# itailang/SampleNet

Measured on AMD Instinct MI355X. Metric: point-clouds/sec fwd+bwd, Bx1024->64 soft-proj+Chamfer, higher is better.
Workload: dtype f32; 1 GPU; BASELINE configs[1]: SampleNet sampler train step (fwd + simplification/projection losses + bwd), B=32 per GPU, 1024->64 points, K=8, bottleneck 128; no optimizer step; batch_per_gpu=32, global_batch=32, n_in=1024, n_out=64, group_size=8, parallelism=dp1, rccl_ranks=0, grad_allreduce=none, execution=whole step replayed as one hipGraph

## Files before the change

### include/samplenet_hip_internal.h

```cpp
#ifndef SAMPLENET_HIP_INTERNAL_H
#define SAMPLENET_HIP_INTERNAL_H

#include "samplenet_hip.h"

#ifdef __cplusplus
extern "C" {
#endif

int sn_sampler_loss_forward(int nproj, const float *proj, const float *lsimp, const float *temperature,
                            float alpha, float lmbda, float min_sigma, float *loss, sn_stream_t stream);
int sn_sampler_loss_backward(int nproj, const float *grad_loss, const float *temperature, float alpha, float lmbda,
                             float min_sigma, float *grad_proj, float *grad_lsimp, float *grad_T, sn_stream_t stream);

int sn_pairscan_colmin_splits(int B, int N, int M);
int sn_pairscan_forward_partial(int B, int N, int M, int K, const float *P, int p_layout, const float *Q, int q_layout,
                                int *knn_idx, float *dist_q, int *idx_q, float *proj, int proj_layout,
                                const float *temperature, float min_sigma, void *workspace, long long workspace_bytes,
                                sn_stream_t stream);
int sn_pairscan_forward_partial_fc(int B, int N, int M, int K, const float *P, int p_layout, const float *fc_z,
                                   const float *fc_scale, const float *fc_shift, const float *fc_w, const float *fc_bias,
                                   int Kfc, float *q_out, int *knn_idx, float *dist_q, int *idx_q, float *proj,
                                   int proj_layout, const float *temperature, float min_sigma, void *workspace,
                                   long long workspace_bytes, sn_stream_t stream);
int sn_sampler_step_loss_forward(int B, int M, int N, int G, const float *dist_q, const void *colmin_ws, const float *proj,
                                 const float *temperature, float alpha, float lmbda, float weight, float min_sigma,
                                 float *dist_p, int *idx_p, int *argmax1, float *partial, float *loss, int defer_value,
                                 sn_stream_t stream);
int sn_sampler_step_loss_forward_direct(int B, int M, int N, const float *dist_q, const float *dist_p, const float *proj,
                                        const float *temperature, float alpha, float lmbda, float weight, float min_sigma,
                                        int *argmax1, float *partial, float *loss, int defer_value, sn_stream_t stream);
int sn_sampler_step_loss_backward(int B, int N, int M, int K, const float *P, int p_layout, const float *Q,
                                  const int *knn_idx, const int *idx_q, const int *idx_p, const int *argmax1,
                                  const float *temperature, float min_sigma, float alpha, float lmbda, float weight,
                                  const float *grad_loss, float *grad_Q, float *gsig_scratch, float *grad_T,
                                  const float *deferred_partial, float *deferred_loss, sn_stream_t stream);
int sn_pairscan_forward_keys(int B, int N, int M, int K, const float *P, int p_layout, float *Q, const float *fc_z,
                             const float *fc_scale, const float *fc_shift, const float *fc_w, const float *fc_bias, int Kfc,
                             int *knn_idx, float *dist_q, int *idx_q, float *proj, int proj_layout, const float *temperature,
                             float min_sigma, void *colmin_keys, float *qpart, void *qmax, sn_stream_t stream);
int sn_sampler_step_loss_keys(int B, int N, int M, int K, const float *P, int p_layout, const float *Q, const int *knn_idx,
                              const int *idx_q, void *colmin_keys, const float *qpart, const void *qmax, int G,
                              const float *temperature, float min_sigma, float alpha, float lmbda, float weight,
                              const float *grad_loss, float *grad_Q, float *gsig_scratch, float *grad_T, float *dpsum,
                              float *loss, sn_stream_t stream, void *deferred_tail, const float *grad_proj,
                              const float *grad_sigma);
int sn_surface_values_keys(int B, int N, int M, int G, const void *colmin_keys, const float *qpart, const void *qmax,
                           const float *temperature, float min_sigma, float weight, const float *y_bcn, float *simp_bnc,
                           float *dpsum, float *values, sn_stream_t stream);
int sn_surface_gather_upstream(int nproj, const float *g_lsimp, const float *g_sigma, const float *g_proj, float *scalars,
                               float *proj_out, sn_stream_t stream);
int sn_conv_stack_set_persist_min_tiles(int tiles);
int sn_fps_set_variant(int v);
int sn_step_tail_bytes(void);
int sn_step_tail_set_error_words(void *tail_blob, const void *fwd_sync, const void *bwd_sync);


int sn_layer_forward_bn(int R, int Ci, int Co, const float *ain, const float *coef_prev, const float *W,
                        const float *bias, float *z, float *stats, const float *gamma, const float *beta,
                        float eps, float momentum, float *running_mean, float *running_var,
                        long long *num_batches_tracked, float *coef, sn_stream_t stream);
int sn_conv_forward_bn_pool(int R, int Ci, int Co, int npts, const float *ain, const float *coef_prev, const float *W,
                            const float *bias, float *z, float *stats, const float *gamma, const float *beta, float eps,
                            float momentum, float *running_mean, float *running_var, long long *num_batches_tracked,
                            float *coef, float *pool_val, int *pool_idx, float *pooled, int *argsel, float *zsel,
                            sn_stream_t stream);
int sn_conv_stack_forward_supported(int B, int N, int nlayers, const int *channels);
long long sn_conv_stack_acc_elems(int nlayers);
int sn_conv_stack_z1_free_supported(int B, int N, int nlayers, const int *channels);
long long sn_conv_stack_acc_sum_elems(int nlayers, const int *channels);
int sn_conv_stack_forward_bn(int B, int N, int nlayers, const int *channels, const float *x, const float *const *W,
                             const float *const *bias, const float *const *gamma, const float *const *beta,
                             float *const *running_mean, float *const *running_var, long long *const *num_batches_tracked,
                             const float *eps, const float *momentum, float *const *z, float *const *coef, long long *acc,
                             float *pool_val, int *pool_idx, float *pooled, int *argsel, float *zsel, sn_stream_t stream);
long long sn_conv_stack_backward_scratch_floats(int B, int N, int nlayers, const int *channels);
int sn_conv_stack_backward(int B, int N, int nlayers, const int *channels, const float *x, const float *const *W,
                           const float *bias0, const float *const *z, const float *const *coef, const float *gsel,
                           const int *argsel, const float *kcoef_top, long long *acc, float *scratch, float *const *dW,
                           float *const *dgamma, float *const *dbeta, float *const *dbias, const void *step_tail,
                           sn_stream_t stream);
int sn_layer_backward(int R, int Ci, int Co, int dz_mode, const float *dy, const float *z, const float *kcoef,
                      const float *gsel, const int *argsel, int npts, const float *W, const float *zprev,
                      const float *coef_prev, float *dyprev, float *stats, float *part, float *dW, float *db,
                      float *prev_dgamma, float *prev_dbeta, float *prev_dbias, float *prev_kcoef, long long prev_bn_rows,
// ... 220 lines not shown
```

### samplenet_amd/csrc/pointnet_mlp.hip

```cpp
#include "mlp_host.h"

namespace sn {

template <class T, bool FULL, int AMODE, int KT = 0, bool PLANES = false, bool IN3A = false>
__global__ void __launch_bounds__(T::THREADS) __attribute__((amdgpu_waves_per_eu(T::THREADS / 128, 8))) linear_fwd_kernel(FwdArgs g)
{
    extern __shared__ __attribute__((aligned(16))) float lds[];
    SN_TL(0);
    SN_TL_ID(0);
    const int row0 = blockIdx.x * T::BM, col0 = blockIdx.y * T::BN;
    const int R = g.a.rows, Co = g.w.co, Ci = g.w.ci;
    f32x16 acc[T::TM][T::TN];
#pragma unroll
    for (int i = 0; i < T::TM; ++i)
#pragma unroll
        for (int j = 0; j < T::TN; ++j)
#pragma unroll
            for (int e = 0; e < 16; ++e) acc[i][j][e] = 0.f;
    const ActSrc a = g.a;
    const WSrc w = g.w;
    const int lane = threadIdx.x & 63;
    const int wave = __builtin_amdgcn_readfirstlane(threadIdx.x >> 6);
    const int wr = wave / T::WC, wc = wave % T::WC;
    float biasv[T::TN];
// ... 1465 lines not shown
    return 1;
}

[[maybe_unused]] constexpr long long kWPlaneLL = (long long)128 * 128 * 3 * 2 / 8;
[[maybe_unused]] constexpr long long kWPlaneWideLL = (long long)256 * 256 * 3 * 2 / 8;
static bool conv_stack_wide(int nlayers, const int *channels)
{
    for (int l = 1; l <= nlayers; ++l)
        if (channels[l] > kFxRow) return true;
    return false;
}
extern "C" int sn_conv_stack_z1_free_supported(int B, int N, int nlayers, const int *channels)
{
#if SN_BF16X3
    if (!sn_conv_stack_forward_supported(B, N, nlayers, channels) || nlayers < 3 || nlayers - 1 > 4) return 0;
    if (channels[1] != 64 || channels[2] != 64) return 0;
    long long nb = 0;
    for (int l = 1; l < nlayers; ++l) nb += ((long long)channels[l] * channels[l + 1] + 1023) / 1024;
    return nb <= (long long)B * N / 64 ? 1 : 0;
#else
    return 0;
#endif
}
extern "C" long long sn_conv_stack_acc_sum_elems(int nlayers, const int *channels)
{
    if (nlayers <= 0) return 0;
    return (long long)nlayers * ((channels && conv_stack_wide(nlayers, channels)) ? 2 : 1) * kFxLayer;
}
extern "C" long long sn_conv_stack_acc_elems(int nlayers)
{
    return nlayers > 0 ? (long long)nlayers * 2 * kFxLayer + (long long)(nlayers - 1) * kWPlaneWideLL : 0;
}

static int g_persist_min_tiles = 4;
static int g_in3_blocks = 0;
extern "C" int sn_conv_stack_set_in3_blocks(int blocks)
{
    const int prev = g_in3_blocks;
    g_in3_blocks = blocks < 0 ? 0 : blocks;
    return prev;
}
extern "C" int sn_conv_stack_set_persist_min_tiles(int tiles)
{
    const int old = g_persist_min_tiles;
    g_persist_min_tiles = tiles;
    return old;
}
template <class TT, int KT, bool IN3A>
static int launch_fwd_persist(const FwdArgs &g, int ntiles, int tpw, int nwg, hipStream_t st)
{
    const size_t lds = sizeof(float) * ((size_t)(KT / BKX) * 3 * TT::BM * LDX + 2 * KT + (size_t)2 * TT::WR * 2 * TT::BN + (size_t)TT::WR * TT::WC * 16 * 36);
    static SnLdsAttr attr;
    if (sn_lds_attr(attr, (const void *)linear_fwd_persist_kernel<TT, KT, IN3A, 2>, lds, "linear_fwd_persist_kernel")) return SN_ERR_UNSUPPORTED;
    hipLaunchKernelGGL((linear_fwd_persist_kernel<TT, KT, IN3A, 2>), dim3(nwg), dim3(TT::THREADS), lds, st, g, ntiles, tpw);
    return 0;
}

template <class TT, int KT>
static void launch_fwd_fx(const FwdArgs &g, dim3 grid, size_t lds, hipStream_t st)
{
    if (g.wplanes)
        hipLaunchKernelGGL((linear_fwd_kernel<TT, true, ACT_BN_RELU_FX, KT, SN_BF16X3 != 0>), grid, dim3(TT::THREADS), lds, st, g);
    else
        hipLaunchKernelGGL((linear_fwd_kernel<TT, true, ACT_BN_RELU_FX, KT>), grid, dim3(TT::THREADS), lds, st, g);
}

extern "C" int sn_conv_stack_forward_bn(int B, int N, int nlayers, const int *channels, const float *x, const float *const *W,
                                        const float *const *bias, const float *const *gamma, const float *const *beta,
                                        float *const *running_mean, float *const *running_var,
                                        long long *const *num_batches_tracked, const float *eps, const float *momentum,
                                        float *const *z, float *const *coef, long long *acc, float *pool_val, int *pool_idx,
                                        float *pooled, int *argsel, float *zsel, sn_stream_t stream)
{
    if (!sn_conv_stack_forward_supported(B, N, nlayers, channels))
        return sn_set_error(SN_ERR_UNSUPPORTED, "sn_conv_stack_forward_bn: needs N % 64 == 0 and 64 / 128 (/ 256 inside the stack) channels");
    SN_REQUIRE(x && W && gamma && beta && eps && momentum && z && coef && acc && pool_val && pool_idx, "null pointer");
    SN_REQUIRE((pooled && argsel && zsel) || (!pooled && !argsel && !zsel), "pooled / argsel / zsel: all or none");
    hipStream_t st = (hipStream_t)stream;
// ... 27 lines not shown
        if (nb > R / 64) job.n = 0;
    }
#endif
    const bool keys_pool = !pooled || (B > 32 && N >= 128 && channels[nlayers] <= 128);
    if (keys_pool) {
        job.zero_keys = reinterpret_cast<unsigned long long *>(pool_val), job.nkeys = B * 2 * channels[nlayers];
        SN_REQUIRE((long long)job.nkeys <= (long long)(R / 64) * 256, "too few rows to clear the pool keys");
    }
    int in3_nb = 1;
    {
        const long long need = std::max<long long>(job.n > 0 ? job.first[job.n] : 0, keys_pool ? (job.nkeys + 255) / 256 : 0);
        while (in3_nb < 8 && (R / 64) / (in3_nb * 2) >= std::max<long long>(need, 4 * device_cus()) && (R / 64) % (in3_nb * 2) == 0) in3_nb *= 2;
        if (g_in3_blocks > 0 && (R / 64) / g_in3_blocks >= std::max<long long>(need, 1)) in3_nb = g_in3_blocks;
    }
    hipLaunchKernelGGL(conv_in3_fwd_kernel, dim3((R / 64 + in3_nb - 1) / in3_nb, channels[1] / 64), dim3(256), 0, st, R, channels[1], x, W[0],
                       bias ? bias[0] : nullptr, z[0], (float *)nullptr, acc, acc + (size_t)(nlayers - 1) * S + kFxPoison, job,
                       in3_nb);
    using T = TileBig;
    for (int l = 1; l < nlayers; ++l) {
        const int Ci = channels[l], Co = channels[l + 1];
        FwdArgs g = make_fwd(R, Ci, Co, z[l - 1], nullptr, W[l], bias ? bias[l] : nullptr, z[l], nullptr);
        g.acc_in = acc + (size_t)(l - 1) * S, g.bn_prev = bn_of(l - 1), g.acc_out = acc + (size_t)l * S;
        if (l >= 2) g.zero_ptr = acc + (size_t)(l - 2) * S, g.zero_n = (int)S;
        if (l == nlayers - 1) {
            g.pool_npts = N;
            if (!keys_pool) g.pool_val = pool_val, g.pool_idx = pool_idx;
            else g.pool_keys = reinterpret_cast<unsigned long long *>(pool_val);
        }
        g.wplanes = job.n > 0 ? planes[l] : nullptr;
        const bool pl = g.wplanes != nullptr;
#if SN_BF16X3
        if (pl && g.z && (l < nlayers - 1 || keys_pool) && (l > 1 || z1free) && (Ci == 64 || Co == 128) && Ci <= 128 && Co <= 128 && R % 64 == 0) {
            const int ntiles = R / 64, per_cu = Co == 128 ? 1 : 2, nmax = device_cus() * per_cu;
            if (g_persist_min_tiles > 0 && ntiles >= g_persist_min_tiles * nmax) {
                const int tpw = (ntiles + nmax - 1) / nmax, nwg = (ntiles + tpw - 1) / tpw;
                if (l == 1) g.x3 = x, g.w3 = W[0], g.b3 = bias ? bias[0] : nullptr;
                int rc = 0;
                const bool ht = Co == 128 && l != 1;
                const int nmax_h = device_cus() * 2, tpw_h = 2 * ((ntiles + nmax_h - 1) / nmax_h), nwg_h = (2 * ntiles + tpw_h - 1) / tpw_h;
                using THT = Tile<32, 128, 1, 4>;
                if (l == 1) rc = launch_fwd_persist<T, 64, true>(g, ntiles, tpw, nwg, st);
                else if (ht && Ci == 128) rc = launch_fwd_persist<THT, 128, false>(g, 2 * ntiles, tpw_h, nwg_h, st);
                else if (ht) rc = launch_fwd_persist<THT, 64, false>(g, 2 * ntiles, tpw_h, nwg_h, st);
                else rc = launch_fwd_persist<T, 64, false>(g, ntiles, tpw, nwg, st);
                if (rc) return rc;
                continue;
            }
        }
#endif
        if (l == 1 && z1free) {
            SN_REQUIRE(pl, "z[0] == NULL: the weight planes are missing");
            g.x3 = x, g.w3 = W[0], g.b3 = bias ? bias[0] : nullptr;
            const dim3 grid(R / T::BM, Co / T::BN);
            const size_t lds = shaped_lds(lds_bytes<T>() + (size_t)2 * Ci * sizeof(float), grid);
            hipLaunchKernelGGL((linear_fwd_kernel<T, true, ACT_BN_RELU_FX, 64, SN_BF16X3 != 0, SN_BF16X3 != 0>), grid, dim3(T::THREADS), lds, st, g);
            continue;
        }
        if (Co % 128 == 0) {
            using TW = TileWide;
            const dim3 grid(R / TW::BM, Co / TW::BN);
            const size_t lds = shaped_lds(lds_bytes<TW>() + (size_t)2 * Ci * sizeof(float), grid);
            if (Ci == 256) {
                SN_REQUIRE(pl, "a 256-channel input needs the pre-split weight planes");
                hipLaunchKernelGGL((linear_fwd_kernel<TW, true, ACT_BN_RELU_FX, 256, SN_BF16X3 != 0>), grid, dim3(TW::THREADS), lds, st, g);
            } else if (Ci == 128 && pl) launch_fwd_fx<TW, 128>(g, grid, lds, st);
            else if (Ci == 128) launch_fwd_fx<TW, 0>(g, grid, lds, st);
            else launch_fwd_fx<TW, 64>(g, grid, lds, st);
// ... 125 lines not shown
```

### samplenet_amd/csrc/pointnet_mlp_backward.hip

```cpp
#include "mlp_host.h"

namespace sn {

struct DgradArgs {
    DzSrc dz;
    WSrc w;
    ActSrc prev;
    float *dyprev;
    float *stats;
    BnBwd bb;
};

template <class T, bool FULL, int ZMODE, int PMODE>
__device__ __forceinline__ void dgrad_body(const DgradArgs &g, int bx, int by, float *lds)
{
    SN_TL(0);
    SN_TL_ID(2);
    const int row0 = bx * T::BM, col0 = by * T::BN;
    const int R = g.dz.rows, Co = g.w.co, Ci = g.w.ci;
    f32x16 acc[T::TM][T::TN];
#pragma unroll
    for (int i = 0; i < T::TM; ++i)
#pragma unroll
        for (int j = 0; j < T::TN; ++j)
// ... 612 lines not shown
        if (IN3) st[5 * CI + tid] = tid < 9 ? red[RB * NST * CI + tid] : 0.f;
    }
    SN_TL_DRAIN();
    SN_TL(7);
}

typedef short s16x4 __attribute__((ext_vector_type(4)));
typedef short s16x8 __attribute__((ext_vector_type(8)));
typedef __attribute__((address_space(3))) s16x4 lds_s16x4;
__device__ __forceinline__ bf16x8 lds_tr8(const __bf16 *p, int pitch)
{
    const s16x4 lo = __builtin_amdgcn_ds_read_tr16_b64_v4i16((lds_s16x4 *)(p));
    const s16x4 hi = __builtin_amdgcn_ds_read_tr16_b64_v4i16((lds_s16x4 *)(p + 4 * pitch));
    const s16x8 v = {lo[0], lo[1], lo[2], lo[3], hi[0], hi[1], hi[2], hi[3]};
    return __builtin_bit_cast(bf16x8, v);
}

__device__ __forceinline__ bf16x8 lds_tr8_2(const __bf16 *plo, const __bf16 *phi)
{
    const s16x4 lo = __builtin_amdgcn_ds_read_tr16_b64_v4i16((lds_s16x4 *)(plo));
    const s16x4 hi = __builtin_amdgcn_ds_read_tr16_b64_v4i16((lds_s16x4 *)(phi));
    const s16x8 v = {lo[0], lo[1], lo[2], lo[3], hi[0], hi[1], hi[2], hi[3]};
    return __builtin_bit_cast(bf16x8, v);
}

template <int CI, int CO>
struct CbxShape {
    static constexpr int TR = CO == 128 ? 32 : 64;
    static constexpr int KS = (CI == 64 && CO == 128) ? 2 : 1;
    static constexpr bool SWZ = CO == 128;
    static constexpr int LDZ = SWZ ? 160 : CO + 8, LDP = SWZ ? (CI == 128 ? 160 : 96) : CI + 8;
    static constexpr int ZPL = TR * LDZ, PPL = TR * LDP;
    static constexpr int BUF = 3 * (ZPL + PPL);
    static constexpr int TSZ = 4 * 32 * 36;
    static constexpr int XSZ = 2 * 3 * TR;
    static constexpr size_t TOFF = (size_t)2 * BUF * 2;
    static constexpr size_t LDS_BYTES = TOFF + TSZ * sizeof(float);
    static constexpr size_t LDS_BYTES_IN3 = LDS_BYTES + (XSZ + 4 * CI) * sizeof(float);
    static_assert(LDS_BYTES_IN3 <= 160 * 1024, "tile buffers exceed the LDS");
};

template <int CO, int CI, int TR, int ZMODE, bool FULLR, int NZ4>
__device__ __forceinline__ void cbx_stage(const ConvBwdArgs &g, int tile, int n0, int tid, __bf16 *__restrict__ Zb,
                                          const float4 (&rz)[NZ4], const float4 (&rdy)[NZ4], const int4 &rag, const float4 &rgs,
                                          const float4 &k1, const float4 &k2, const float4 &k3)
{
    constexpr int ZSTEP = 256 / (CO / 4);
    constexpr int LDZ = CbxShape<CI, CO>::LDZ;
    const int R = g.dz.rows;
    const int row0 = tile * TR;
    const int zc4 = (tid % (CO / 4)) * 4, zr = tid / (CO / 4);
#pragma unroll
    for (int q = 0; q < NZ4; ++q) {
        const int rt = zr + q * ZSTEP;
        float4 d;
        if (ZMODE == DZ_POOL) {
            const int n = n0 + rt;
            d.x = rag.x == n ? rgs.x : 0.f;
            d.y = rag.y == n ? rgs.y : 0.f;
            d.z = rag.z == n ? rgs.z : 0.f;
            d.w = rag.w == n ? rgs.w : 0.f;
        } else {
            d = rdy[q];
        }
        float4 v = make_float4(fmaf(k1.x, d.x, fmaf(k2.x, rz[q].x, k3.x)), fmaf(k1.y, d.y, fmaf(k2.y, rz[q].y, k3.y)),
                               fmaf(k1.z, d.z, fmaf(k2.z, rz[q].z, k3.z)), fmaf(k1.w, d.w, fmaf(k2.w, rz[q].w, k3.w)));
        if (!FULLR) {
            const float m = row0 + rt < R ? 1.f : 0.f;
            v.x *= m, v.y *= m, v.z *= m, v.w *= m;
        }
        stage_split_p<TR * LDZ, LDZ>(Zb, rt, CbxShape<CI, CO>::SWZ ? zc4 ^ (((rt >> 2) & 3) << 3) : zc4, v);
    }
}

template <int CI, int CO, int ZMODE, bool FULLR, bool IN3 = false, bool RZ1 = false, int GZ = CO, int GP = CI, int GW = CI, int DM = 0>
__global__ void __launch_bounds__(512) conv_bwd_bx3_kernel(ConvBwdArgs g)
{
    static_assert(DM == 0 || (!IN3 && CbxShape<CI, CO>::KS == 1), "two-pass modes: plain 128 x 128 tiles");
    static_assert(!RZ1 || IN3, "RZ1: the layer below must be the xyz layer");
    using S = CbxShape<CI, CO>;
    static_assert(!IN3 || (S::TR == 64 && ZMODE == DZ_BN), "IN3: 64-row tiles (one row per lane for the moments)");
    constexpr int NST = IN3 ? 5 : 2;
    constexpr int TR = S::TR, LDZ = S::LDZ, LDP = S::LDP, ZPL = S::ZPL, PPL = S::PPL, BUF = S::BUF;
    constexpr int NZ4 = TR * CO / 4 / 256, NP4 = TR * CI / 4 / 256;
    constexpr int NCB = CI / 32, NOB = CO / 32, RB = TR / 32;
    constexpr int KS = S::KS;
    constexpr bool kSkew = !IN3 && CI == 128 && CO == 128;
    constexpr int NDW = RB * NCB * KS;
    constexpr int NWT = NOB * NCB / 4;
    constexpr int KD = CO / 16 / KS, KW = TR / 16;
    static_assert((CI == 64 || CI == 128) && (CO == 64 || CO == 128), "instantiated for 64 / 128 channels");
    static_assert(NDW == 4 && NZ4 >= 1 && NP4 >= 1 && NWT >= 1, "wave roles below assume four dgrad waves per row tile");
    extern __shared__ __attribute__((aligned(16))) float lds[];
    __bf16 *Lb = reinterpret_cast<__bf16 *>(lds);
    float *Tf = reinterpret_cast<float *>(reinterpret_cast<char *>(lds) + S::TOFF);

    const int tid = threadIdx.x, lane = tid & 63, l31 = lane & 31, h = lane >> 5;
    const int wave = __builtin_amdgcn_readfirstlane(tid >> 6);
    float *Ts = Tf + (wave & 3) * (32 * 36);
    float *Xs = Tf + S::TSZ;
    const int R = g.dz.rows;
    const bool do_d = wave < 4;
    const int dwv = wave & 3;
    const int dt = dwv / KS, kh = dwv % KS;
    const int rb = dt % RB, cb = dt / RB;
    const int q0 = dwv * NWT;
    const int cob = q0 / NCB;
    const int G = gridDim.x;
    const int tile0 = blockIdx.x, tend = g.ntiles, tst = G;

    SN_TL(0);
#ifdef SN_TIMELINE
    sn_hw_record();
#endif
    if (do_d) {
        const int zc4 = (tid % (CO / 4)) * 4, pc4 = (tid % (CI / 4)) * 4;
        const bool fxin = ZMODE == DZ_BN && g.acc_in != nullptr;
        float4 k1 = make_float4(0.f, 0.f, 0.f, 0.f), k2 = k1, k3 = k1;
        if (!fxin) {
            k1 = *reinterpret_cast<const float4 *>(g.dz.k1 + zc4);
            k2 = *reinterpret_cast<const float4 *>(g.dz.k2 + zc4);
            k3 = *reinterpret_cast<const float4 *>(g.dz.k3 + zc4);
        }
        const float scd = g.scale_prev[cb * 32 + l31], shd = g.shift_prev[cb * 32 + l31];
        const unsigned qvo = ((rb * 32 + 4 * h) * GP + cb * 32 + l31) * 4;
        const unsigned ovo = ((rb * 32 + (lane >> 3)) * GP + cb * 32 + (lane & 7) * 4) * 4;
        const unsigned zvo = ((tid / (CO / 4)) * GZ + zc4) * 4, pvo = ((tid / (CI / 4)) * GP + pc4) * 4, avo = zc4 * 4;
        CbfRsrc rs;
        rs.z = make_rsrc(g.dz.z, (unsigned)R * GZ * 4);
        rs.dy = make_rsrc(ZMODE == DZ_BN ? g.dz.dy : g.dz.z, (unsigned)R * GZ * 4);
        rs.zprev = make_rsrc(g.zprev, (unsigned)R * GP * 4);
        rs.dyprev = make_rsrc(g.dyprev, (unsigned)R * GP * 4);
        rs.dyacc = make_rsrc(DM == 2 ? (const void *)g.dyacc : (const void *)g.zprev, (unsigned)R * GP * 4);
        const unsigned nclouds = ZMODE == DZ_POOL ? (unsigned)((R + g.dz.npts - 1) / g.dz.npts) : 1u;
        rs.argsel = make_rsrc(ZMODE == DZ_POOL ? (const void *)g.dz.argsel : (const void *)g.dz.z, nclouds * CO * 4);
        rs.gsel = make_rsrc(ZMODE == DZ_POOL ? (const void *)g.dz.gsel : (const void *)g.dz.z, nclouds * CO * 4);
        const sn_rsrc rsx = make_rsrc(IN3 ? (const void *)g.xin : (const void *)g.dz.z, (unsigned)R * 12);
        const bool xthr = IN3 && tid < 3 * TR / 4;
        int xslot[4];
#pragma unroll
        for (int j = 0; j < 4; ++j) {
            const int i = tid * 4 + j;
            xslot[j] = (i % 3) * TR + i / 3;
        }
        float4 rx = make_float4(0.f, 0.f, 0.f, 0.f);
        float gx0 = 0.f, gx1 = 0.f, gx2 = 0.f;
        float mom[9];
#pragma unroll
        for (int k = 0; k < 9; ++k) mom[k] = 0.f;
        const int tpc = ZMODE == DZ_POOL ? g.dz.npts / TR : 1;
        const int bstep = tst / tpc, tstep = tst - bstep * tpc;
        int cloud = tile0 / tpc, tic = tile0 - cloud * tpc;
        float4 rz[NZ4], rdy[NZ4], rp[NP4];
        int4 rag = make_int4(0, 0, 0, 0);
        float4 rgs = make_float4(0.f, 0.f, 0.f, 0.f);
        float s0 = 0.f, s1 = 0.f;
        float4 *W3s = reinterpret_cast<float4 *>(Xs + S::XSZ);
        if (RZ1 && tid < CI)
            W3s[tid] = make_float4(g.w_in[tid * 3], g.w_in[tid * 3 + 1], g.w_in[tid * 3 + 2], g.b_in ? g.b_in[tid] : 0.f);
        float4 vout[4];
#pragma unroll
        for (int i = 0; i < 4; ++i) vout[i] = make_float4(0.f, 0.f, 0.f, 0.f);

        int tile = tile0;
        cbf_issue_loads<CO, CI, TR, ZMODE, NZ4, NP4, true, GZ, GP>(rs, tile, cloud, zvo, pvo, avo, rz, rdy, rp, rag, rgs);
        if (xthr) rx = buf_load4(rsx, (unsigned)tid * 16, (unsigned)tile * (TR * 12));
        float wraw[KD][8];
#pragma unroll
        for (int kk = 0; kk < KD; ++kk)
#pragma unroll
            for (int t = 0; t < 8; ++t) wraw[kk][t] = g.W[(size_t)((kh * KD + kk) * 16 + 8 * h + t) * GW + cb * 32 + l31];
        if (fxin) {
            const float *Ks = Tf;
            __syncthreads();
            k1 = *reinterpret_cast<const float4 *>(Ks + zc4);
            k2 = *reinterpret_cast<const float4 *>(Ks + CO + zc4);
            k3 = *reinterpret_cast<const float4 *>(Ks + 2 * CO + zc4);
        }
        cbx_stage<CO, CI, TR, ZMODE, FULLR, NZ4>(g, tile, tic * TR, tid, Lb, rz, rdy, rag, rgs, k1, k2, k3);
        if (xthr) Xs[xslot[0]] = rx.x, Xs[xslot[1]] = rx.y, Xs[xslot[2]] = rx.z, Xs[xslot[3]] = rx.w;
        bf16x8 wf[KD][3];
#pragma unroll
        for (int kk = 0; kk < KD; ++kk)
#pragma unroll
            for (int t = 0; t < 8; ++t) {
                __bf16 h1, h2, h3;
                split3(wraw[kk][t], h1, h2, h3);
                wf[kk][0][t] = h1, wf[kk][1][t] = h2, wf[kk][2][t] = h3;
            }
        __syncthreads();
        for (int it = 0; tile < tend; ++it, tile += tst) {
            const __bf16 *Zb = Lb + (it & 1) * BUF;
            const auto store_prev = [&]() __attribute__((always_inline)) {
                if (!IN3 && it > 0 && kh == 0) {
                    const unsigned oso = (unsigned)(tile - tst) * (TR * GP * 4);
#pragma unroll
                    for (int i = 0; i < 4; ++i) buf_store4<SN_ST_DY>(vout[i], rs.dyprev, ovo, oso + i * (8 * GP * 4));
                }
            };
            store_prev();
            float zq[16], pq[16];
            if (!RZ1 && DM != 1 && (KS == 1 || kh == 0))
#pragma unroll
                for (int e = 0; e < 16; ++e)
                    zq[e] = buf_load1(rs.zprev, qvo, (unsigned)tile * (TR * GP * 4) + ((e & 3) + 8 * (e >> 2)) * (GP * 4));
            if (DM == 2)
#pragma unroll
                for (int e = 0; e < 16; ++e)
                    pq[e] = buf_load1(rs.dyacc, qvo, (unsigned)tile * (TR * GP * 4) + ((e & 3) + 8 * (e >> 2)) * (GP * 4));
            const bool more = tile + tst < tend;
            const int nxt = more ? tile + tst : tile;
            int ncloud = cloud, ntic = tic;
            if (more) {
                ncloud += bstep, ntic += tstep;
                if (ntic >= tpc) ntic -= tpc, ++ncloud;
            }
            cbf_issue_loads<CO, CI, TR, ZMODE, NZ4, NP4, true, GZ, GP>(rs, nxt, ncloud, zvo, pvo, avo, rz, rdy, rp, rag, rgs);
            if (xthr) rx = buf_load4(rsx, (unsigned)tid * 16, (unsigned)nxt * (TR * 12));
            __builtin_amdgcn_sched_barrier(0);
            if (it == 1) SN_TL(5);

            f32x16 acc;
#pragma unroll
            for (int e = 0; e < 16; ++e) acc[e] = 0.f;
            const int fsw = S::SWZ ? ((l31 >> 2) & 3) ^ h : 0;
            const __bf16 *apr = Zb + (rb * 32 + l31) * LDZ + kh * KD * 16;
            const __bf16 *ape = S::SWZ ? apr + (fsw << 3) : apr + 8 * h, *apo = S::SWZ ? apr + ((fsw ^ 2) << 3) : apr + 8 * h + 16;
#pragma unroll
            for (int kk = 0; kk < KD; ++kk) {
                const __bf16 *ap = ((kk & 1) ? apo : ape) + (kk >> 1) * 32;
                const bf16x8 a0 = *reinterpret_cast<const bf16x8 *>(ap);
                const bf16x8 a1 = *reinterpret_cast<const bf16x8 *>(ap + ZPL);
                const bf16x8 a2 = *reinterpret_cast<const bf16x8 *>(ap + 2 * ZPL);
                acc = __builtin_amdgcn_mfma_f32_32x32x16_bf16(a0, wf[kk][2], acc, 0, 0, 0);
                acc = __builtin_amdgcn_mfma_f32_32x32x16_bf16(a2, wf[kk][0], acc, 0, 0, 0);
                acc = __builtin_amdgcn_mfma_f32_32x32x16_bf16(a1, wf[kk][1], acc, 0, 0, 0);
                acc = __builtin_amdgcn_mfma_f32_32x32x16_bf16(a0, wf[kk][1], acc, 0, 0, 0);
                acc = __builtin_amdgcn_mfma_f32_32x32x16_bf16(a1, wf[kk][0], acc, 0, 0, 0);
                acc = __builtin_amdgcn_mfma_f32_32x32x16_bf16(a0, wf[kk][0], acc, 0, 0, 0);
            }
            if (it == 1) SN_TL(1);
            if (kSkew) __syncthreads();
            if (KS == 2) {
                float *Tx = Tf + (dwv | 1) * (32 * 36);
                if (kh == 1)
#pragma unroll
                    for (int e = 0; e < 16; ++e) Tx[e * 64 + lane] = acc[e];
                __syncthreads();
                if (kh == 0)
#pragma unroll
                    for (int e = 0; e < 16; ++e) acc[e] += Tx[e * 64 + lane];
            }
            if (kh == 0) {
                if (RZ1) {
#pragma clang fp contract(off)
                    const float4 wd = W3s[cb * 32 + l31];
                    const float w3d0 = wd.x, w3d1 = wd.y, w3d2 = wd.z, b3d = wd.w;
                    const float *xq = Xs + (it & 1) * (3 * TR) + rb * 32 + 4 * h;
#pragma unroll
                    for (int q = 0; q < 4; ++q) {
                        const float4 x0 = *reinterpret_cast<const float4 *>(xq + 8 * q);
                        const float4 x1 = *reinterpret_cast<const float4 *>(xq + TR + 8 * q);
                        const float4 x2 = *reinterpret_cast<const float4 *>(xq + 2 * TR + 8 * q);
                        zq[4 * q + 0] = fmaf(w3d2, x2.x, fmaf(w3d1, x1.x, w3d0 * x0.x)) + b3d;
                        zq[4 * q + 1] = fmaf(w3d2, x2.y, fmaf(w3d1, x1.y, w3d0 * x0.y)) + b3d;
                        zq[4 * q + 2] = fmaf(w3d2, x2.z, fmaf(w3d1, x1.z, w3d0 * x0.z)) + b3d;
                        zq[4 * q + 3] = fmaf(w3d2, x2.w, fmaf(w3d1, x1.w, w3d0 * x0.w)) + b3d;
                    }
                }
#pragma unroll
                for (int e = 0; e < 16; ++e) {
                    if (DM == 1) {
                        Ts[frag_row(e, lane) * 36 + l31] = acc[e];
                        continue;
                    }
                    const float z = zq[e];
                    const float a = DM == 2 ? acc[e] + pq[e] : acc[e];
                    const float v = fmaf(z, scd, shd) > 0.f ? a : 0.f;
                    s0 += v;
                    s1 = fmaf(v, z, s1);
                    if (IN3) acc[e] = v;
                    if (!IN3) Ts[frag_row(e, lane) * 36 + l31] = v;
                }
                if (IN3) {
                    const float *Xc = Xs + (it & 1) * (3 * TR);
                    const float *xp = Xc + rb * 32 + 4 * h;
#pragma unroll
                    for (int q = 0; q < 4; ++q) {
                        const float4 x0 = *reinterpret_cast<const float4 *>(xp + 8 * q);
                        const float4 x1 = *reinterpret_cast<const float4 *>(xp + TR + 8 * q);
                        const float4 x2 = *reinterpret_cast<const float4 *>(xp + 2 * TR + 8 * q);
                        gx0 = fmaf(acc[4 * q + 3], x0.w, fmaf(acc[4 * q + 2], x0.z, fmaf(acc[4 * q + 1], x0.y, fmaf(acc[4 * q], x0.x, gx0))));
                        gx1 = fmaf(acc[4 * q + 3], x1.w, fmaf(acc[4 * q + 2], x1.z, fmaf(acc[4 * q + 1], x1.y, fmaf(acc[4 * q], x1.x, gx1))));
                        gx2 = fmaf(acc[4 * q + 3], x2.w, fmaf(acc[4 * q + 2], x2.z, fmaf(acc[4 * q + 1], x2.y, fmaf(acc[4 * q], x2.x, gx2))));
                    }
                    if (wave == 0) {
                        const float a = Xc[lane], b = Xc[TR + lane], c = Xc[2 * TR + lane];
                        mom[0] += a, mom[1] += b, mom[2] += c;
                        mom[3] = fmaf(a, a, mom[3]), mom[4] = fmaf(a, b, mom[4]), mom[5] = fmaf(a, c, mom[5]);
                        mom[6] = fmaf(b, b, mom[6]), mom[7] = fmaf(b, c, mom[7]), mom[8] = fmaf(c, c, mom[8]);
                    }
                }
// ... 39 lines not shown
#pragma unroll
                for (int k = 0; k < 9; ++k) {
                    float m = mom[k];
#pragma unroll
                    for (int o = 32; o >= 1; o >>= 1) m += __shfl_xor(m, o);
                    if (lane == 0) red[RB * NST * CI + k] = m;
                }
            }
        }
    } else {
        constexpr int PSTEPW = 256 / (CI / 4);
        const int tw = tid - 256;
        const int pc4w = (tw % (CI / 4)) * 4, prw = tw / (CI / 4);
        const unsigned pvow = (prw * GP + pc4w) * 4;
        const sn_rsrc rzp = make_rsrc(g.zprev, (unsigned)R * GP * 4);
        float4 rpw[NP4];
        float4 scw = make_float4(0.f, 0.f, 0.f, 0.f), shw = scw;
        const sn_rsrc rsxw = make_rsrc(IN3 ? (const void *)g.xin : (const void *)g.dz.z, (unsigned)R * 12);
        const unsigned xvow = prw * 12;
        float4 w3w[4];
#pragma unroll
        for (int j = 0; j < 4; ++j) w3w[j] = make_float4(0.f, 0.f, 0.f, 0.f);
        if (RZ1) {
#pragma unroll
            for (int j = 0; j < 4; ++j)
                w3w[j] = make_float4(g.w_in[(pc4w + j) * 3], g.w_in[(pc4w + j) * 3 + 1], g.w_in[(pc4w + j) * 3 + 2], g.b_in ? g.b_in[pc4w + j] : 0.f);
        }
        auto load_p = [&](int t) __attribute__((always_inline)) {
#pragma unroll
            for (int q = 0; q < NP4; ++q)
                rpw[q] = RZ1 ? buf_load3(rsxw, xvow, (unsigned)t * (TR * 12) + q * (PSTEPW * 12))
                             : buf_load4(rzp, pvow, (unsigned)t * (TR * GP * 4) + q * (PSTEPW * GP * 4));
        };
        auto stage_p = [&](__bf16 *Pb) __attribute__((always_inline)) {
#pragma unroll
            for (int q = 0; q < NP4; ++q) {
                float4 zp = rpw[q];
                if (RZ1) {
#pragma clang fp contract(off)
                    const float x0 = rpw[q].x, x1 = rpw[q].y, x2 = rpw[q].z;
                    zp.x = fmaf(w3w[0].z, x2, fmaf(w3w[0].y, x1, w3w[0].x * x0)) + w3w[0].w;
                    zp.y = fmaf(w3w[1].z, x2, fmaf(w3w[1].y, x1, w3w[1].x * x0)) + w3w[1].w;
                    zp.z = fmaf(w3w[2].z, x2, fmaf(w3w[2].y, x1, w3w[2].x * x0)) + w3w[2].w;
                    zp.w = fmaf(w3w[3].z, x2, fmaf(w3w[3].y, x1, w3w[3].x * x0)) + w3w[3].w;
                }
                const float4 a = make_float4(relu_np(fmaf(zp.x, scw.x, shw.x)), relu_np(fmaf(zp.y, scw.y, shw.y)),
                                             relu_np(fmaf(zp.z, scw.z, shw.z)), relu_np(fmaf(zp.w, scw.w, shw.w)));
                stage_split_p<TR * LDP, LDP>(Pb, prw + q * PSTEPW, pc4w, a);
            }
        };
        load_p(tile0);
        scw = *reinterpret_cast<const float4 *>(g.scale_prev + pc4w);
        shw = *reinterpret_cast<const float4 *>(g.shift_prev + pc4w);
        if (ZMODE == DZ_BN && g.acc_in != nullptr) {
            float *Ks = Tf;
            const int c = tid - 256;
            if (c < CO) {
                const BnBwd bb = g.bb_in;
                double su, sz;
                fx_get2<kFxShiftBwd>(g.acc_in, c, su, sz);
                const BnBwdOut o = bn_backward_coefs(bb.R, su, sz, bn_bwd_inputs(bb, CO, c));
                Ks[c] = o.k1, Ks[CO + c] = o.k2, Ks[2 * CO + c] = o.k3;
                if (blockIdx.x == 0) {
                    bb.dgamma[c] = o.dgamma, bb.dbeta[c] = o.dbeta;
                    if (bb.dbias) bb.dbias[c] = o.dbias;
                    if (bb.kcoef) bb.kcoef[c] = o.k1, bb.kcoef[CO + c] = o.k2, bb.kcoef[2 * CO + c] = o.k3;
                }
            }
            fx_clear_share(g.zero_ptr, g.zero_n, blockIdx.x, gridDim.x, tid - 256, 256);
            __syncthreads();
        }
        f32x16 accw[NWT];
#pragma unroll
        for (int n = 0; n < NWT; ++n)
#pragma unroll
            for (int e = 0; e < 16; ++e) accw[n][e] = 0.f;
        stage_p(Lb + 3 * ZPL);
        if (kSkew) load_p(tile0 + tst < tend ? tile0 + tst : tile0);
        __syncthreads();
        const int trr = 8 * h + ((lane & 15) >> 2), trc = 16 * ((lane >> 4) & 1) + 4 * (lane & 3);
        int tile = tile0;
        for (int it = 0; tile < tend; ++it, tile += tst) {
            const __bf16 *Zb = Lb + (it & 1) * BUF, *Pb = Zb + 3 * ZPL;
            const bool more = tile + tst < tend;
            if (kSkew) {
                if (more) stage_p(Lb + ((it + 1) & 1) * BUF + 3 * ZPL);
                if (it == 1) SN_TL(2);
                __syncthreads();
                if (it == 1) SN_TL(3);
                load_p(tile + 2 * tst < tend ? tile + 2 * tst : tile);
                __builtin_amdgcn_sched_barrier(0);
            } else {
                load_p(more ? tile + tst : tile);
                __builtin_amdgcn_sched_barrier(0);
            }
            const __bf16 *ap = Zb + trr * LDZ + (S::SWZ ? (cob * 32 + trc) ^ ((2 * h) << 3) : cob * 32 + trc);
            const __bf16 *aph = Zb + (trr + 4) * LDZ + (S::SWZ ? (cob * 32 + trc) ^ ((2 * h + 1) << 3) : cob * 32 + trc);
            const __bf16 *bp = Pb + trr * LDP + trc;
            bf16x8 fa[2][3], fb[2][3][NWT];
            auto frag_load = [&](int kk, int s) __attribute__((always_inline)) {
#pragma unroll
                for (int p = 0; p < 3; ++p) {
                    fa[s][p] = lds_tr8_2(ap + p * ZPL + kk * 16 * LDZ, aph + p * ZPL + kk * 16 * LDZ);
#pragma unroll
                    for (int n = 0; n < NWT; ++n) fb[s][p][n] = lds_tr8(bp + p * PPL + kk * 16 * LDP + ((q0 + n) % NCB) * 32, LDP);
                }
            };
            frag_load(0, 0);
#pragma unroll
            for (int kk = 0; kk < KW; ++kk) {
                if (kk + 1 < KW) frag_load(kk + 1, (kk + 1) & 1);
                __builtin_amdgcn_sched_barrier(0);
                const bf16x8(&a)[3] = fa[kk & 1];
                const bf16x8(&b)[3][NWT] = fb[kk & 1];
#define SN_BX3_TERM(PA, PB) \
    _Pragma("unroll") for (int n = 0; n < NWT; ++n) accw[n] = __builtin_amdgcn_mfma_f32_32x32x16_bf16(a[PA], b[PB][n], accw[n], 0, 0, 0)
                SN_BX3_TERM(0, 2);
                SN_BX3_TERM(2, 0);
                SN_BX3_TERM(1, 1);
                SN_BX3_TERM(0, 1);
                SN_BX3_TERM(1, 0);
                SN_BX3_TERM(0, 0);
#undef SN_BX3_TERM
                __builtin_amdgcn_sched_barrier(0);
            }
            if (it == 1) SN_TL(1);
            if (KS == 2) __syncthreads();
            if (!kSkew && more) stage_p(Lb + ((it + 1) & 1) * BUF + 3 * ZPL);
            __syncthreads();
            if (it == 1) SN_TL(4);
        }
        SN_TL(6);
        const int pld = g.part_ld > 0 ? g.part_ld : CI;
        const float *P = g.part + (size_t)blockIdx.x * (g.part_wg_stride > 0 ? g.part_wg_stride : CO * CI);
        const sn_rsrc rpart = make_rsrc(P, (unsigned)((CO - 1) * pld + CI) * 4);
        const unsigned wvo = ((lane >> 3) * pld + (lane & 7) * 4) * 4;
        float *Tw = lds + RB * NST * CI + 16 + (wave - 4) * (32 * 36);
#pragma unroll
        for (int n = 0; n < NWT; ++n) {
            const int colb = ((q0 + n) % NCB) * 32;
#pragma unroll
            for (int e = 0; e < 16; ++e) Tw[frag_row(e, lane) * 36 + l31] = accw[n][e];
#pragma unroll
            for (int i = 0; i < 4; ++i) {
                const int rt = 8 * i + (lane >> 3);
                buf_store4<SN_ST_PART>(*reinterpret_cast<const float4 *>(Tw + rt * 36 + (lane & 7) * 4), rpart, wvo,
                                       (unsigned)((cob * 32 + 8 * i) * pld + colb) * 4);
            }
        }
    }
    __syncthreads();
    if (tid < CI && DM != 1) {
        const float *red = lds;
        const int sld = g.stats_ld > 0 ? g.stats_ld : CI;
        const sn_rsrc rst = make_rsrc(g.stats + (size_t)blockIdx.x * (IN3 ? 6 : 2) * sld, (unsigned)(IN3 ? 6 : 2) * sld * 4);
#pragma unroll
        for (int k = 0; k < NST; ++k) {
            float a = red[k * CI + tid];
            if (RB == 2) a += red[(NST + k) * CI + tid];
            if (!IN3 && g.acc_out)
                fx_add<kFxShiftBwd>(g.acc_out, blockIdx.x % kFxSlots, k, tid, a);
// ... 1239 lines not shown
```

Before: 187,700 point-clouds/s.

## Share staged pre-activation tiles via LDS and add per-shape persistent routing thresholds

The backward fused kernel previously re-read the previous layer's pre-activation z from global memory, or recomputed it from xyz and the input weights for the first layer. Now the weight-gradient waves, which already load and stage that data, also write the fp32 tile into a double-buffered LDS region, and the data-gradient waves read it from there. This removes a global load and the RZ1 recompute in exchange for twice the transpose scratch LDS and extra LDS stores. The forward path also replaces one global persistent-kernel tile threshold with per-shape defaults (2,2,3,6), so different layers can be routed to the persistent kernel at different sizes.

```diff
diff --git a/include/samplenet_hip_internal.h b/include/samplenet_hip_internal.h
--- a/include/samplenet_hip_internal.h
+++ b/include/samplenet_hip_internal.h
@@ -50,6 +50,7 @@
 int sn_surface_gather_upstream(int nproj, const float *g_lsimp, const float *g_sigma, const float *g_proj, float *scalars,
                                float *proj_out, sn_stream_t stream);
 int sn_conv_stack_set_persist_min_tiles(int tiles);
+int sn_conv_stack_set_persist_min_tiles_shape(int Ci, int Co, int first, int tiles);
 int sn_fps_set_variant(int v);
 int sn_step_tail_bytes(void);
 int sn_step_tail_set_error_words(void *tail_blob, const void *fwd_sync, const void *bwd_sync);
diff --git a/samplenet_amd/csrc/pointnet_mlp.hip b/samplenet_amd/csrc/pointnet_mlp.hip
--- a/samplenet_amd/csrc/pointnet_mlp.hip
+++ b/samplenet_amd/csrc/pointnet_mlp.hip
@@ -1521,7 +1521,24 @@
     return nlayers > 0 ? (long long)nlayers * 2 * kFxLayer + (long long)(nlayers - 1) * kWPlaneWideLL : 0;
 }
 
-static int g_persist_min_tiles = 4;
+enum { kPersistDefault = -1, kPersistAlways = -2 };
+enum { kShapeIn3, kShape64x64, kShape64x128, kShape128x128, kPersistShapes };
+static const int kPersistBuiltin[kPersistShapes] = {2, 2, 3, 6};
+static int g_persist_shape[kPersistShapes] = {2, 2, 3, 6};
+static int g_persist_min_tiles = kPersistDefault;
+static int persist_shape_of(int Ci, int Co, bool first)
+{
+    if (first) return Ci == 64 && Co == 64 ? kShapeIn3 : -1;
+    if (Ci == 64) return Co == 64 ? kShape64x64 : Co == 128 ? kShape64x128 : -1;
+    return Ci == 128 && Co == 128 ? kShape128x128 : -1;
+}
+static bool persist_route(int Ci, int Co, bool first, int ntiles, int nmax)
+{
+    const int s = persist_shape_of(Ci, Co, first);
+    if (s < 0) return false;
+    const int mt = g_persist_min_tiles != kPersistDefault ? g_persist_min_tiles : g_persist_shape[s];
+    return mt == kPersistAlways || (mt > 0 && (long long)ntiles >= (long long)mt * nmax);
+}
 static int g_in3_blocks = 0;
 extern "C" int sn_conv_stack_set_in3_blocks(int blocks)
 {
@@ -1532,7 +1549,15 @@
 extern "C" int sn_conv_stack_set_persist_min_tiles(int tiles)
 {
     const int old = g_persist_min_tiles;
-    g_persist_min_tiles = tiles;
+    g_persist_min_tiles = tiles < kPersistAlways ? kPersistDefault : tiles;
+    return old;
+}
+extern "C" int sn_conv_stack_set_persist_min_tiles_shape(int Ci, int Co, int first, int tiles)
+{
+    const int s = persist_shape_of(Ci, Co, first != 0);
+    if (s < 0 || tiles < kPersistAlways) return kPersistDefault;
+    const int old = g_persist_shape[s];
+    g_persist_shape[s] = tiles == kPersistDefault ? kPersistBuiltin[s] : tiles;
     return old;
 }
 template <class TT, int KT, bool IN3A>
@@ -1626,7 +1651,7 @@
 #if SN_BF16X3
         if (pl && g.z && (l < nlayers - 1 || keys_pool) && (l > 1 || z1free) && (Ci == 64 || Co == 128) && Ci <= 128 && Co <= 128 && R % 64 == 0) {
             const int ntiles = R / 64, per_cu = Co == 128 ? 1 : 2, nmax = device_cus() * per_cu;
-            if (g_persist_min_tiles > 0 && ntiles >= g_persist_min_tiles * nmax) {
+            if (persist_route(Ci, Co, l == 1, ntiles, nmax)) {
                 const int tpw = (ntiles + nmax - 1) / nmax, nwg = (ntiles + tpw - 1) / tpw;
                 if (l == 1) g.x3 = x, g.w3 = W[0], g.b3 = bias ? bias[0] : nullptr;
                 int rc = 0;
diff --git a/samplenet_amd/csrc/pointnet_mlp_backward.hip b/samplenet_amd/csrc/pointnet_mlp_backward.hip
--- a/samplenet_amd/csrc/pointnet_mlp_backward.hip
+++ b/samplenet_amd/csrc/pointnet_mlp_backward.hip
@@ -668,11 +668,11 @@
     static constexpr int LDZ = SWZ ? 160 : CO + 8, LDP = SWZ ? (CI == 128 ? 160 : 96) : CI + 8;
     static constexpr int ZPL = TR * LDZ, PPL = TR * LDP;
     static constexpr int BUF = 3 * (ZPL + PPL);
-    static constexpr int TSZ = 4 * 32 * 36;
+    static constexpr int TSET = 4 * 32 * 36, TSZ = 2 * TSET;
     static constexpr int XSZ = 2 * 3 * TR;
     static constexpr size_t TOFF = (size_t)2 * BUF * 2;
     static constexpr size_t LDS_BYTES = TOFF + TSZ * sizeof(float);
-    static constexpr size_t LDS_BYTES_IN3 = LDS_BYTES + (XSZ + 4 * CI) * sizeof(float);
+    static constexpr size_t LDS_BYTES_IN3 = LDS_BYTES + XSZ * sizeof(float);
     static_assert(LDS_BYTES_IN3 <= 160 * 1024, "tile buffers exceed the LDS");
 };
 
@@ -733,7 +733,6 @@
 
     const int tid = threadIdx.x, lane = tid & 63, l31 = lane & 31, h = lane >> 5;
     const int wave = __builtin_amdgcn_readfirstlane(tid >> 6);
-    float *Ts = Tf + (wave & 3) * (32 * 36);
     float *Xs = Tf + S::TSZ;
     const int R = g.dz.rows;
     const bool do_d = wave < 4;
@@ -750,7 +749,7 @@
     sn_hw_record();
 #endif
     if (do_d) {
-        const int zc4 = (tid % (CO / 4)) * 4, pc4 = (tid % (CI / 4)) * 4;
+        const int zc4 = (tid % (CO / 4)) * 4;
         const bool fxin = ZMODE == DZ_BN && g.acc_in != nullptr;
         float4 k1 = make_float4(0.f, 0.f, 0.f, 0.f), k2 = k1, k3 = k1;
         if (!fxin) {
@@ -761,7 +760,7 @@
         const float scd = g.scale_prev[cb * 32 + l31], shd = g.shift_prev[cb * 32 + l31];
         const unsigned qvo = ((rb * 32 + 4 * h) * GP + cb * 32 + l31) * 4;
         const unsigned ovo = ((rb * 32 + (lane >> 3)) * GP + cb * 32 + (lane & 7) * 4) * 4;
-        const unsigned zvo = ((tid / (CO / 4)) * GZ + zc4) * 4, pvo = ((tid / (CI / 4)) * GP + pc4) * 4, avo = zc4 * 4;
+        const unsigned zvo = ((tid / (CO / 4)) * GZ + zc4) * 4, avo = zc4 * 4;
         CbfRsrc rs;
         rs.z = make_rsrc(g.dz.z, (unsigned)R * GZ * 4);
         rs.dy = make_rsrc(ZMODE == DZ_BN ? g.dz.dy : g.dz.z, (unsigned)R * GZ * 4);
@@ -791,15 +790,12 @@
         int4 rag = make_int4(0, 0, 0, 0);
         float4 rgs = make_float4(0.f, 0.f, 0.f, 0.f);
         float s0 = 0.f, s1 = 0.f;
-        float4 *W3s = reinterpret_cast<float4 *>(Xs + S::XSZ);
-        if (RZ1 && tid < CI)
-            W3s[tid] = make_float4(g.w_in[tid * 3], g.w_in[tid * 3 + 1], g.w_in[tid * 3 + 2], g.b_in ? g.b_in[tid] : 0.f);
         float4 vout[4];
 #pragma unroll
         for (int i = 0; i < 4; ++i) vout[i] = make_float4(0.f, 0.f, 0.f, 0.f);
 
         int tile = tile0;
-        cbf_issue_loads<CO, CI, TR, ZMODE, NZ4, NP4, true, GZ, GP>(rs, tile, cloud, zvo, pvo, avo, rz, rdy, rp, rag, rgs);
+        cbf_issue_loads<CO, CI, TR, ZMODE, NZ4, NP4, true, GZ, GP>(rs, tile, cloud, zvo, 0u, avo, rz, rdy, rp, rag, rgs);
         if (xthr) rx = buf_load4(rsx, (unsigned)tid * 16, (unsigned)tile * (TR * 12));
         float wraw[KD][8];
 #pragma unroll
@@ -807,7 +803,7 @@
 #pragma unroll
             for (int t = 0; t < 8; ++t) wraw[kk][t] = g.W[(size_t)((kh * KD + kk) * 16 + 8 * h + t) * GW + cb * 32 + l31];
         if (fxin) {
-            const float *Ks = Tf;
+            const float *Ks = Tf + S::TSET;
             __syncthreads();
             k1 = *reinterpret_cast<const float4 *>(Ks + zc4);
             k2 = *reinterpret_cast<const float4 *>(Ks + CO + zc4);
@@ -835,11 +831,11 @@
                 }
             };
             store_prev();
+            float *Ts = Tf + (it & 1) * S::TSET + dwv * (32 * 36);
             float zq[16], pq[16];
-            if (!RZ1 && DM != 1 && (KS == 1 || kh == 0))
-#pragma unroll
-                for (int e = 0; e < 16; ++e)
-                    zq[e] = buf_load1(rs.zprev, qvo, (unsigned)tile * (TR * GP * 4) + ((e & 3) + 8 * (e >> 2)) * (GP * 4));
+            if (DM != 1 && (KS == 1 || kh == 0))
+#pragma unroll
+                for (int e = 0; e < 16; ++e) zq[e] = Ts[frag_row(e, lane) * 36 + l31];
             if (DM == 2)
 #pragma unroll
                 for (int e = 0; e < 16; ++e)
@@ -851,7 +847,7 @@
                 ncloud += bstep, ntic += tstep;
                 if (ntic >= tpc) ntic -= tpc, ++ncloud;
             }
-            cbf_issue_loads<CO, CI, TR, ZMODE, NZ4, NP4, true, GZ, GP>(rs, nxt, ncloud, zvo, pvo, avo, rz, rdy, rp, rag, rgs);
+            cbf_issue_loads<CO, CI, TR, ZMODE, NZ4, NP4, true, GZ, GP>(rs, nxt, ncloud, zvo, 0u, avo, rz, rdy, rp, rag, rgs);
             if (xthr) rx = buf_load4(rsx, (unsigned)tid * 16, (unsigned)nxt * (TR * 12));
             __builtin_amdgcn_sched_barrier(0);
             if (it == 1) SN_TL(5);
@@ -878,7 +874,7 @@
             if (it == 1) SN_TL(1);
             if (kSkew) __syncthreads();
             if (KS == 2) {
-                float *Tx = Tf + (dwv | 1) * (32 * 36);
+                float *Tx = Tf + (it & 1) * S::TSET + (dwv | 1) * (32 * 36);
                 if (kh == 1)
 #pragma unroll
                     for (int e = 0; e < 16; ++e) Tx[e * 64 + lane] = acc[e];
@@ -888,22 +884,6 @@
                     for (int e = 0; e < 16; ++e) acc[e] += Tx[e * 64 + lane];
             }
             if (kh == 0) {
-                if (RZ1) {
-#pragma clang fp contract(off)
-                    const float4 wd = W3s[cb * 32 + l31];
-                    const float w3d0 = wd.x, w3d1 = wd.y, w3d2 = wd.z, b3d = wd.w;
-                    const float *xq = Xs + (it & 1) * (3 * TR) + rb * 32 + 4 * h;
-#pragma unroll
-                    for (int q = 0; q < 4; ++q) {
-                        const float4 x0 = *reinterpret_cast<const float4 *>(xq + 8 * q);
-                        const float4 x1 = *reinterpret_cast<const float4 *>(xq + TR + 8 * q);
-                        const float4 x2 = *reinterpret_cast<const float4 *>(xq + 2 * TR + 8 * q);
-                        zq[4 * q + 0] = fmaf(w3d2, x2.x, fmaf(w3d1, x1.x, w3d0 * x0.x)) + b3d;
-                        zq[4 * q + 1] = fmaf(w3d2, x2.y, fmaf(w3d1, x1.y, w3d0 * x0.y)) + b3d;
-                        zq[4 * q + 2] = fmaf(w3d2, x2.z, fmaf(w3d1, x1.z, w3d0 * x0.z)) + b3d;
-                        zq[4 * q + 3] = fmaf(w3d2, x2.w, fmaf(w3d1, x1.w, w3d0 * x0.w)) + b3d;
-                    }
-                }
 #pragma unroll
                 for (int e = 0; e < 16; ++e) {
                     if (DM == 1) {
@@ -1009,7 +989,7 @@
                 rpw[q] = RZ1 ? buf_load3(rsxw, xvow, (unsigned)t * (TR * 12) + q * (PSTEPW * 12))
                              : buf_load4(rzp, pvow, (unsigned)t * (TR * GP * 4) + q * (PSTEPW * GP * 4));
         };
-        auto stage_p = [&](__bf16 *Pb) __attribute__((always_inline)) {
+        auto stage_p = [&](__bf16 *Pb, float *Sr) __attribute__((always_inline)) {
 #pragma unroll
             for (int q = 0; q < NP4; ++q) {
                 float4 zp = rpw[q];
@@ -1021,6 +1001,10 @@
                     zp.z = fmaf(w3w[2].z, x2, fmaf(w3w[2].y, x1, w3w[2].x * x0)) + w3w[2].w;
                     zp.w = fmaf(w3w[3].z, x2, fmaf(w3w[3].y, x1, w3w[3].x * x0)) + w3w[3].w;
                 }
+                if (DM != 1) {
+                    const int rt = prw + q * PSTEPW;
+                    *reinterpret_cast<float4 *>(Sr + (((rt >> 5) + RB * (pc4w >> 5)) * KS) * (32 * 36) + (rt & 31) * 36 + (pc4w & 31)) = zp;
+                }
                 const float4 a = make_float4(relu_np(fmaf(zp.x, scw.x, shw.x)), relu_np(fmaf(zp.y, scw.y, shw.y)),
                                              relu_np(fmaf(zp.z, scw.z, shw.z)), relu_np(fmaf(zp.w, scw.w, shw.w)));
                 stage_split_p<TR * LDP, LDP>(Pb, prw + q * PSTEPW, pc4w, a);
@@ -1030,7 +1014,7 @@
         scw = *reinterpret_cast<const float4 *>(g.scale_prev + pc4w);
         shw = *reinterpret_cast<const float4 *>(g.shift_prev + pc4w);
         if (ZMODE == DZ_BN && g.acc_in != nullptr) {
-            float *Ks = Tf;
+            float *Ks = Tf + S::TSET;
             const int c = tid - 256;
             if (c < CO) {
                 const BnBwd bb = g.bb_in;
@@ -1052,7 +1036,7 @@
         for (int n = 0; n < NWT; ++n)
 #pragma unroll
             for (int e = 0; e < 16; ++e) accw[n][e] = 0.f;
-        stage_p(Lb + 3 * ZPL);
+        stage_p(Lb + 3 * ZPL, Tf);
         if (kSkew) load_p(tile0 + tst < tend ? tile0 + tst : tile0);
         __syncthreads();
         const int trr = 8 * h + ((lane & 15) >> 2), trc = 16 * ((lane >> 4) & 1) + 4 * (lane & 3);
@@ -1061,7 +1045,7 @@
             const __bf16 *Zb = Lb + (it & 1) * BUF, *Pb = Zb + 3 * ZPL;
             const bool more = tile + tst < tend;
             if (kSkew) {
-                if (more) stage_p(Lb + ((it + 1) & 1) * BUF + 3 * ZPL);
+                if (more) stage_p(Lb + ((it + 1) & 1) * BUF + 3 * ZPL, Tf + ((it + 1) & 1) * S::TSET);
                 if (it == 1) SN_TL(2);
                 __syncthreads();
                 if (it == 1) SN_TL(3);
@@ -1103,7 +1087,7 @@
             }
             if (it == 1) SN_TL(1);
             if (KS == 2) __syncthreads();
-            if (!kSkew && more) stage_p(Lb + ((it + 1) & 1) * BUF + 3 * ZPL);
+            if (!kSkew && more) stage_p(Lb + ((it + 1) & 1) * BUF + 3 * ZPL, Tf + ((it + 1) & 1) * S::TSET);
             __syncthreads();
             if (it == 1) SN_TL(4);
         }
```

Result: slower. 185,500 point-clouds/s (-1.2%).
